# msyriac/orphics

Hardware: AMD Instinct MI355X
Metric: QE kappa reconstructions/sec on 8192^2 maps (higher is better)
Workload: dtype f64

## Files before the change

orphics_amd/csrc/common.hpp:

```cpp
#pragma once
#include <hip/hip_runtime.h>
#include <cstdio>
#include <cstring>
#include <string>
#include "../../include/orphics_amd.h"
#include "cx.hpp"

namespace oa {

std::string& last_error_ref();

inline int fail(const std::string& msg) {
    last_error_ref() = msg;
    return 1;
}

#define OA_HIP(expr)                                                                              \
    do {                                                                                          \
        hipError_t _e = (expr);                                                                   \
        if (_e != hipSuccess)                                                                     \
            return ::oa::fail(std::string(#expr) + ": " + hipGetErrorString(_e) + " (" + __FILE__ + \
                              ":" + std::to_string(__LINE__) + ")");                              \
    } while (0)

#define OA_REQUIRE(cond, msg)                         \
    do {                                              \
        if (!(cond)) return ::oa::fail(std::string(msg)); \
    } while (0)

#define OA_LAUNCH_CHECK() OA_HIP(hipGetLastError())

template <typename T, int N>
struct alignas(sizeof(T) * N > 16 ? 16 : sizeof(T) * N) Arr {
    T v[N];
};

struct DivBinFuse {
    const int32_t* ids; long ipitch;
    const int32_t* ids_t;
    const void* fn_t;
    int tab_logc, tab_rows;
    const unsigned long long* run_ent; const int32_t* run_off;
    int run_w, run_rb, run_cap;
    double pnorm; int nids, nxh;
    double* part;
    long part_cap;
    double* sums;
    unsigned* ticket;
    const int64_t* mcounts; int64_t* n; double* S; double* C;
    int store;
    int gx;
    bool done;
};

inline int flat_grid(long units, int block = 256, int cap = 8192) {
    long g = (units + block - 1) / block;
    if (g < 1) g = 1;
    if (g > cap) g = cap;
    return (int)g;
}

}

struct oa_plan {
    int ny, nx, logNy, logNx, dtype, device;
    long kp;
    void* tw_x;
    void* tw_y;
    void* scratch;
    size_t scratch_bytes;
    void* ly;
    void* lx;
    void* lyd;
    void* lxd;
    double* ly64;
    double* lx64;
    bool have_laxes;
    bool pow2;
    oa_plan* inner;
    int My, Mx;
    void* chirp_y; void* chirp_x;
    void* cz_bhat; void* cz_a; void* cz_f;
    void* cz_full;
    bool mixed;
    void* mr_twx; void* mr_twxh; void* mr_twy;
    void* pipe;
    void* rq8c[5];
    void* tw_y_small[16];
    void* tw_y_m3[16];
};

namespace oa {
int plan_ensure_scratch(oa_plan* p, size_t bytes);
int czt_setup(oa_plan* p);
void czt_release(oa_plan* p);
int czt_c2c(oa_plan* p, const void* in, void* out, int inverse, double scale, hipStream_t st);
int czt_r2c(oa_plan* p, const void* real_in, void* hc_out, double scale, hipStream_t st);
int czt_c2r(oa_plan* p, const void* hc_in, void* real_out, double scale, hipStream_t st);
bool mixed_sides_ok(int ny, int nx);
int mixed_setup(oa_plan* p);
void mixed_release(oa_plan* p);
int mixed_c2c(oa_plan* p, const void* in, void* out, int inverse, double scale, hipStream_t st);
int mixed_r2c(oa_plan* p, const void* real_in, void* hc_out, double scale, hipStream_t st);
int mixed_c2r(oa_plan* p, const void* hc_in, void* real_out, double scale, hipStream_t st);
int mixed_c2r_windowed(oa_plan* p, const void* hc_in, void* real_out, double scale, const void* window, hipStream_t st);
int mixed_cols_inverse(oa_plan* p, const void* hc_in, void* hc_out, hipStream_t st);
int mixed_lens_derivs(oa_plan* p, int nmaps, const void* real_in, long in_stride, void* k0, void* hc_pool, void* real_pool, int nd, hipStream_t st,
                      const void* hc_in, long hc_stride, double hc_scale);
void pipeline_release(oa_plan* p);
int n1_pool_reserve(oa_plan* p, size_t bytes, char** out);
long work_pitch(const oa_plan* p, int w);
int bin_power_moments(int dtype, const void* k, double norm, const int32_t* ids, long n, int nids, long hp, int nxh, double* sums,
                      int64_t* counts, void* scratch, int active_cols, int active_rows, unsigned* ticket,
                      const int64_t* mcounts, int64_t* mn, double* S, double* C, hipStream_t st, int nbatch = 1, long kstride = 0);
int stack_add_region(int dtype, const void* x, double* acc, int ny, long kp, int w, int rb, hipStream_t st, int nbatch = 1, long xstride = 0);
int band_rot2(int dtype, const void* c, const void* s, void* q, void* u, int ny, long kp, int w, int rb, hipStream_t st);
int stack_add_region_multi(int dtype, const void* k, long kstride, const void* wt, long wstride, int nest, double* const* acc, double* acc_mv,
                           int ny, long kp, int w, int rb, hipStream_t st);
int grf_mix_teb_to_tqu(oa_plan* p, uint64_t seed, uint64_t sid0, const void* const* cs, const void* rot_c, const void* rot_s, void* const* out,
                       hipStream_t st);
int band_stack_add_multi(int dtype, const void* k, long kstride, const void* wt, long wstride, int nest, double* const* acc, double* acc_mv,
                         int iny, long ipitch, int any, long apitch, int w, int r, hipStream_t st);
size_t rdn0_part_bytes(int ny, int rb, int nids, int B);
int rdn0_tail_check(const char* who, int nids, int B);
int rdn0_tail(int dtype, const void* k, long kstride, int B, int ny, long kp, int nxh, const int32_t* ids, int nids, double pnorm, int w, int rb,
              const int64_t* mcounts, double* part, int64_t* n, double* S, double* C, hipStream_t st);
size_t rdn0mv_scratch_bytes(int ny, int rb, int nspec, int nids);
int rdn0mv_tail_check(const char* who, int nest, bool have_w, int nspec, const int* host_a, const int* host_b, int nids);
int rdn0mv_tail(int dtype, const void* k, long kstride, const void* wt, long wstride, int nest, int nspec, const int* host_a, const int* host_b, int ny,
                long kp, int nxh, const int32_t* ids, int nids, double pnorm, int w, int rb, const int64_t* mcounts, void* scratch, int64_t* n, double* S,
                double* C, hipStream_t st);
// ... 78 lines not shown
```

orphics_amd/csrc/fft.hip:

```cpp
#include <algorithm>
#include <cmath>
#include <vector>
#include "fft_launch.hpp"
#include "fft_r2c_w64.hpp"
#include "fft_r2c_rs4096.hpp"
#include "fft_divbin.hpp"

namespace oa {

template <typename T, int MODE, class SEQ>
__global__ __launch_bounds__(row_maxnt<SEQ>(), waves_per_eu<T>()) void row_fft_kernel(RowArgs<T> a) {
    GpuCtx c{oa_dyn_smem};
    row_fft_body<T, MODE, SEQ>(c, a);
}

#ifndef OA_W64_OCC
#define OA_W64_OCC 1
#endif
__global__ __launch_bounds__(64, OA_W64_OCC) void row_r2c_w64_kernel(RowW64Args a) {
    GpuCtx c{oa_dyn_smem};
    row_r2c_w64_body(c, a);
}

template <typename T, class SEQ, int LR, bool PF>
// ... 387 lines not shown
        if (!ok && !rc) rc = fail("fft: unsupported row length");
    }
    template <typename T>
    void row_qe_pair8(int pairs, int M, const RowQeArgs<T>& a) {
        const bool ok = dispatch_rq8(M, a.win, a.lr, a.chain != nullptr, [&](auto ac, auto nzc, auto lay, auto ch) {
            constexpr int A = decltype(ac)::value;
            if (ch.value && !a.tab) { if (!rc) rc = fail("fft: estimator chains need a table"); return; }
            if (!a.rq8c) { if (!rc) rc = fail("fft: the 8-point row stage needs the constants of its grid"); return; }
            go(row_qe8_kernel<T, A, decltype(nzc)::value, decltype(lay)::value, decltype(ch)::value>, dim3(pairs), 64 * A, rq8_lds_bytes<T, A, decltype(ch)::value>(), a);
        });
        if (!ok && !rc) rc = fail("fft: unsupported row grid / layout for the 8-point row stage");
    }
    template <typename T>
    void row_qe_pair(int grid, int nt, size_t smem, const RowQeArgs<T>& a) {
        const bool ok = dispatch_seq(a.logL, [&](auto seq) {
            using S = decltype(seq);
            if constexpr (seq_logl<S>() >= 10 && seq_logl<S>() <= 13) {
                if (nt != pair_nt<S>()) { if (!rc) rc = fail("fft: pair row stage launched with the wrong workgroup size"); return; }
                dispatch_pair_nz<S>(pair_first_stage_nz(a.logL, S::rget(0), a.win), [&](auto nzc) {
                    if (a.chain) {
                        if constexpr (seq_logl<S>() <= 12) { if (a.lr == 0 && a.tab) go(row_qe_chain_kernel<T, S, decltype(nzc)::value>, dim3(grid), nt, smem, a); else if (!rc) rc = fail("fft: estimator chains need natural-order planes and a table"); }
                        else if (!rc) rc = fail("fft: estimator chains: unsupported row grid");
                    } else
                    if (a.lr == 2) go(row_qe_pair_kernel<T, S, decltype(nzc)::value, 2>, dim3(grid), nt, smem, a);
                    else if (a.lr == 3) {
                        if constexpr (seq_logl<S>() == 11 && sizeof(T) == 8) go(row_qe_pair_kernel<T, S, decltype(nzc)::value, 3>, dim3(grid), nt, smem, a);
                        else if (!rc) rc = fail("fft: the R = 8 layout of the pair row stage is built for float64 on 2048-point row grids");
                    } else if (a.lr == 0) go(row_qe_pair_kernel<T, S, decltype(nzc)::value, 0>, dim3(grid), nt, smem, a);
                    else if (!rc) rc = fail("fft: unsupported R-layout of the pair row stage");
                });
            } else if (!rc) rc = fail("fft: unsupported row grid for the pair row stage");
        });
        if (!ok && !rc) rc = fail("fft: unsupported row grid");
    }
    template <typename T>
    void col_legs(int gx, int gy, int nt, size_t smem, int logL, const ColLegsArgs<T>& a) {
        if (rc) return;
        rc = launch_col_legs<T>(st, gx, gy, nt, smem, logL, a);
    }
    template <typename T>
    void col_legs_sp(int gx, int nt, size_t smem, int logL, const ColLegsArgs<T>& a) {
        if (rc) return;
        rc = launch_col_legs_sp<T>(st, gx, nt, smem, logL, a);
    }
    template <typename T>
    void col_fwdlegs(int gx, int gy, int nt, size_t smem, int logL, const ColFwdLegsArgs<T>& a) {
        if (rc) return;
        rc = launch_col_fwdlegs<T>(st, gx, gy, nt, smem, logL, a);
    }
    template <typename T>
    void col_fwdlegs_cg(int gx, int gy, int nt, size_t smem, int logL, const ColFwdLegsCgArgs<T>& a, int gz = 1) {
        if (rc) return;
        rc = launch_col_fwdlegs_cg<T>(st, gx, gy, nt, smem, logL, a, gz);
    }
    template <typename T>
    void col_div(int gx, int gy, int nt, size_t smem, int logL, const ColDivArgs<T>& a, int gz = 1) {
        const bool ok = dispatch_seq(logL, [&](auto seq) {
            using S = decltype(seq);
            if constexpr (seq_logl<S>() <= 8) {
                if (nt > col_maxnt<S>()) { if (!rc) rc = fail("fft: column workgroup size exceeds its launch bound"); return; }
                go(col_div_kernel<T, S>, dim3(gx, gy, gz), nt, smem, a);
            } else if (!rc) rc = fail("fft: unsupported column sub-length");
        });
        if (!ok && !rc) rc = fail("fft: unsupported column length");
    }
    DivBinFuse* fuse = nullptr;
#define OA_GO_FUSED(K, ...) go_fused(K<__VA_ARGS__, false>, K<__VA_ARGS__, true>, gx, gz, nt, smem, a)
    template <class K, typename T>
    void go_fused(K kern_ids, K kern_runs, int gx, int gz, int nt, size_t smem, ColDivArgs<T> a) {
        const bool tabs = fuse->tab_logc == a.logC && fuse->tab_rows == a.ny;
        const bool runs = tabs && fuse->run_ent && fuse->run_w == a.width && fuse->run_rb == a.rband && fuse->run_cap <= 2 * nt;
        const K kern = runs ? kern_runs : kern_ids;
        if (runs) smem = std::max(smem, divrun_lds_bytes(a.ny, a.logC, nt, sizeof(T) == 8));
        {
            const hipError_t e = ensure_dyn_lds(reinterpret_cast<const void*>(kern), smem);
            if (e != hipSuccess) { rc = fail(std::string("hipFuncSetAttribute: ") + hipGetErrorString(e)); return; }
        }
        fuse->gx = gx;
        if (!fuse->store) a.out = nullptr;
        a.Fn_t = (tabs && a.fn_moff == 0) ? (const T*)fuse->fn_t : nullptr;
        if (!tabs) fuse->ids_t = nullptr;
        hipLaunchKernelGGL(kern, dim3(gx, 1, gz), dim3(nt), smem, st, a, *fuse);
        hipError_t e = hipGetLastError();
        if (e != hipSuccess) rc = fail(std::string("fft launch: ") + hipGetErrorString(e));
        fuse->done = true;
    }
    template <typename T>
    bool col_div_sp(int gx, size_t smem, int logL, const ColDivArgs<T>& a, int gz = 1) {
        if (rc) return true;
        const int lt = Fft2dPlan<T>::div_lt(), nt = (1 << lt) / EPT;
        const bool narrow = lt < (sizeof(T) == 4 ? 14 : 13);
        constexpr int lc11 = sizeof(T) == 4 ? 3 : 2, lc10 = lc11 + 1;
        if (fuse && !a.accumulate && (long)gx * gz * fuse->nids <= fuse->part_cap && (logL == 10 || logL == 11 || (logL == 12 && !narrow)) &&
            (size_t)(nt / 64) * fuse->nids * sizeof(double) <= ((size_t)1 << lt) * sizeof(cx<T>)) {
            if (logL == 12) OA_GO_FUSED(col_div_sp_bin_kernel, T, Seq<16, 16, 16>, lc11 - 1);
            else if (logL == 11 && !narrow) OA_GO_FUSED(col_div_sp_bin_kernel, T, Seq<16, 16, 8>, lc11);
            else if (logL == 10 && !narrow) OA_GO_FUSED(col_div_sp_bin_kernel, T, Seq<16, 16, 4>, lc10);
            else if (logL == 11) OA_GO_FUSED(col_div_sp_bin_kernel, T, Seq<16, 16, 8>, lc11 - 1);
            else OA_GO_FUSED(col_div_sp_bin_kernel, T, Seq<16, 16, 4>, lc10 - 1);
            return true;
        }
        if (logL == 12 && !narrow) { go(col_div_sp_kernel<T, Seq<16, 16, 16>, lc11 - 1>, dim3(gx, 1, gz), nt, smem, a); return true; }
        if (logL == 11 && !narrow) { go(col_div_sp_kernel<T, Seq<16, 16, 8>, lc11>, dim3(gx, 1, gz), nt, smem, a); return true; }
        if (logL == 10 && !narrow) { go(col_div_sp_kernel<T, Seq<16, 16, 4>, lc10>, dim3(gx, 1, gz), nt, smem, a); return true; }
        if (logL == 11) { go(col_div_sp_kernel<T, Seq<16, 16, 8>, lc11 - 1>, dim3(gx, 1, gz), nt, smem, a); return true; }
        if (logL == 10) { go(col_div_sp_kernel<T, Seq<16, 16, 4>, lc10 - 1>, dim3(gx, 1, gz), nt, smem, a); return true; }
        return false;
    }
    template <typename T>
    void col_div3(int gx, size_t smem, int rows, const ColDivArgs<T>& a, int gz = 1) {
        if (rc) return;
        constexpr int lc = sizeof(T) == 4 ? 3 : 2;
        if (rows != 1536 && rows != 768) { rc = fail("fft: unsupported 3 x 2^k divergence grid"); return; }
        const int nt = a.NT;
        if (fuse && !a.accumulate && (long)gx * gz * fuse->nids <= fuse->part_cap &&
            (size_t)(nt / 64) * fuse->nids * sizeof(double) <= ((size_t)rows << a.logC) * sizeof(cx<T>)) {
            if (rows == 1536) OA_GO_FUSED(col_div3_sp_bin_kernel, T, 8, lc);
            else OA_GO_FUSED(col_div3_sp_bin_kernel, T, 7, lc + 1);
            return;
        }
        if (rows == 1536) go(col_div3_sp_kernel<T, 8, lc>, dim3(gx, 1, gz), nt, smem, a);
        else go(col_div3_sp_kernel<T, 7, lc + 1>, dim3(gx, 1, gz), nt, smem, a);
    }
    template <typename T>
    void col_deriv(int gx, int gy, int nt, size_t smem, const ColDerivArgs<T>& a, int nz) {
        const bool ok = dispatch_seq(a.logL, [&](auto seq) {
            using S = decltype(seq);
            if constexpr (seq_logl<S>() <= 8) {
                if (nt > col_maxnt<S>()) { if (!rc) rc = fail("fft: column workgroup size exceeds its launch bound"); return; }
                go(col_deriv_kernel<T, S>, dim3(gx, gy, nz), nt, smem, a);
            } else if (!rc) rc = fail("fft: unsupported column sub-length");
        });
        if (!ok && !rc) rc = fail("fft: unsupported column length");
    }
    template <typename T>
    void col_grf(int gx, int gy, int nt, size_t smem, const GrfColArgs<T>& a, int nz) {
        const bool ok = dispatch_seq(a.logL, [&](auto seq) {
            using S = decltype(seq);
            if constexpr (seq_logl<S>() <= 8) {
                if (nt > col_maxnt<S>()) { if (!rc) rc = fail("fft: column workgroup size exceeds its launch bound"); return; }
                go(col_grf_kernel<T, S>, dim3(gx, gy, nz), nt, smem, a);
            } else if (!rc) rc = fail("fft: unsupported column sub-length");
        });
        if (!ok && !rc) rc = fail("fft: unsupported column length");
    }
    template <typename T>
    void col_mix(int gx, int gy, int nt, size_t smem, const MixColArgs<T>& a, int nz) {
        const bool ok = dispatch_seq(a.logL, [&](auto seq) {
            using S = decltype(seq);
            if constexpr (seq_logl<S>() <= 8 && !(sizeof(T) == 8 && seq_logl<S>() == 8)) {
                if (nt > col_maxnt<S>()) { if (!rc) rc = fail("fft: column workgroup size exceeds its launch bound"); return; }
                go(col_mix_kernel<T, S>, dim3(gx, gy, nz), nt, smem, a);
            } else if (!rc) rc = fail("fft: unsupported column sub-length");
        });
        if (!ok && !rc) rc = fail("fft: unsupported column length");
    }
    template <typename T>
    void col(int gx, int gy, int nt, size_t smem, const ColArgs<T>& a, int nz = 1) {
        const bool ok = dispatch_seq(a.logL, [&](auto seq) {
            using S = decltype(seq);
            if constexpr (seq_logl<S>() <= 8) {
                if (nt > col_maxnt<S>()) { if (!rc) rc = fail("fft: column workgroup size exceeds its launch bound"); return; }
                go(col_fft_kernel<T, S>, dim3(gx, gy, nz), nt, smem, a);
            } else {
                if (!rc) rc = fail("fft: unsupported column sub-length");
            }
// ... 689 lines not shown
```

orphics_amd/csrc/fft_divbin.hpp:

```cpp
#pragma once
#include "fft_launch.hpp"

namespace oa {

#if defined(__HIP_DEVICE_COMPILE__) && !(defined(__gfx942__) || defined(__gfx950__))
#error "DivBinTail: the ticket hand-over relies on gfx942 / gfx950 behaviour (agent-scope relaxed atomic stores are sc1 write-through, stores count in vmcnt)"
#endif

template <int CTRL>
__device__ __forceinline__ double dpp_f64(double v) {
    const unsigned long long u = __builtin_bit_cast(unsigned long long, v);
    const int lo = __builtin_amdgcn_update_dpp(0, (int)(unsigned)u, CTRL, 0xf, 0xf, false);
    const int hi = __builtin_amdgcn_update_dpp(0, (int)(unsigned)(u >> 32), CTRL, 0xf, 0xf, false);
    return __builtin_bit_cast(double, ((unsigned long long)(unsigned)hi << 32) | (unsigned long long)(unsigned)lo);
}
__device__ __forceinline__ double readlane_f64(double v, int lane) {
    const unsigned long long u = __builtin_bit_cast(unsigned long long, v);
    const unsigned lo = (unsigned)__builtin_amdgcn_readlane((int)(unsigned)u, lane);
    const unsigned hi = (unsigned)__builtin_amdgcn_readlane((int)(unsigned)(u >> 32), lane);
    return __builtin_bit_cast(double, ((unsigned long long)hi << 32) | (unsigned long long)lo);
}
__device__ __forceinline__ double wave_total_f64(double v) {
    v += dpp_f64<0xB1>(v);
    v += dpp_f64<0x4E>(v);
    v += dpp_f64<0x141>(v);
    v += dpp_f64<0x140>(v);
    return ((readlane_f64(v, 0) + readlane_f64(v, 16)) + readlane_f64(v, 32)) + readlane_f64(v, 48);
}

template <class Partial>
__device__ __forceinline__ void divbin_handover(const DivBinFuse& f, double* red, Partial partial) {
    __shared__ int s_last;
    const int t = threadIdx.x, nt = blockDim.x, nids = f.nids;
    const long wg = (long)blockIdx.z * gridDim.x + blockIdx.x;
    for (int i = t; i < nids; i += nt) {
        const double s = partial(i);
        __hip_atomic_store(f.part + wg * nids + i, s, __ATOMIC_RELAXED, __HIP_MEMORY_SCOPE_AGENT);
    }
    asm volatile("s_waitcnt vmcnt(0)" ::: "memory");
    __syncthreads();
    if (t == 0)
        s_last = (__hip_atomic_fetch_add(f.ticket, 1u, OA_TICKET_ORDER, __HIP_MEMORY_SCOPE_AGENT) == gridDim.x * gridDim.z - 1) ? 1 : 0;
    __syncthreads();
    if (!s_last) return;
    const int d = nids - 2;
    int NI = 1;
    while (NI < nids && NI < nt) NI <<= 1;
    const int G = nt / NI > 0 ? nt / NI : 1, gi = t / NI, ii = t - gi * NI;
    const int gx = (int)gridDim.x;
    for (int z = 0; z < (int)gridDim.z; ++z) {
        for (int i0 = 0; i0 < nids; i0 += NI) {
            const int i = i0 + ii;
            __syncthreads();
            if (gi < G) {
                double s = 0.0;
                if (i < nids) {
                    const double* pz = f.part + ((long)z * gx) * nids + i;
                    int b = gi;
                    for (; b + 3 * G < gx; b += 4 * G) {
                        const double p0 = __hip_atomic_load(pz + (long)b * nids, __ATOMIC_RELAXED, __HIP_MEMORY_SCOPE_AGENT);
                        const double p1 = __hip_atomic_load(pz + (long)(b + G) * nids, __ATOMIC_RELAXED, __HIP_MEMORY_SCOPE_AGENT);
                        const double p2 = __hip_atomic_load(pz + (long)(b + 2 * G) * nids, __ATOMIC_RELAXED, __HIP_MEMORY_SCOPE_AGENT);
                        const double p3 = __hip_atomic_load(pz + (long)(b + 3 * G) * nids, __ATOMIC_RELAXED, __HIP_MEMORY_SCOPE_AGENT);
                        s += (p0 + p1) + (p2 + p3);
                    }
                    for (; b < gx; b += G) s += __hip_atomic_load(pz + (long)b * nids, __ATOMIC_RELAXED, __HIP_MEMORY_SCOPE_AGENT);
                }
                red[gi * NI + ii] = s;
            }
            __syncthreads();
            double tot = 0.0;
            if (gi == 0 && i < nids) {
                for (int k = 0; k < G; ++k) tot += red[k * NI + ii];
                f.sums[(long)z * nids + i] = tot;
            }
            __syncthreads();
            if (gi == 0 && i >= 1 && i <= d) red[G * NI + i - 1] = tot / (double)f.mcounts[i];
        }
        __syncthreads();
        const double* bv = red + G * NI;
        if (f.S) {
            for (int a = t; a < d; a += nt) f.S[a] += bv[a];
            for (long e = t; e < (long)d * d; e += nt) {
                const int ra = (int)(e / d), cb = (int)(e - (long)ra * d);
                f.C[e] += bv[ra] * bv[cb];
            }
        }
    }
    if (t == 0) {
        if (f.n) f.n[0] += (int64_t)gridDim.z;
        __hip_atomic_store(f.ticket, 0u, __ATOMIC_RELAXED, __HIP_MEMORY_SCOPE_AGENT);
    }
}

template <typename T>
struct DivBinTail {
    static constexpr bool active = true, needs_ids = true;
    DivBinFuse f;
    double* rows = nullptr;

    __device__ __forceinline__ void begin(GpuCtx&, void* lds, int, int, int) {
        rows = reinterpret_cast<double*>(lds);
        const int nw = blockDim.x >> 6;
        for (int i = threadIdx.x; i < nw * f.nids; i += blockDim.x) rows[i] = 0.0;
    }
    __device__ __forceinline__ int id_at(unsigned yfull, int col) const { return f.ids[(long)yfull * f.ipitch + col]; }
    __device__ __forceinline__ bool packed_ids() const { return f.ids_t != nullptr; }
    __device__ __forceinline__ int id_at_t(long i) const { return f.ids_t[i]; }
    __device__ __forceinline__ void add(GpuCtx&, int id, T pw, int col, int) {
        const int m = (col == 0 || col == f.nxh) ? 1 : (col < f.nxh ? 2 : 0);
        const bool ok = id >= 0 && id < f.nids && m > 0;
        const double v = ok ? (double)(pw * (T)f.pnorm) * (double)m : 0.0;
        const int lane = threadIdx.x & 63;
        double* row = rows + (threadIdx.x >> 6) * f.nids;
        unsigned long long act = __ballot(ok);
        while (act) {
            const int leader = __ffsll((long long)act) - 1;
            const int lid = __shfl(id, leader, 64);
            const bool mine = ok && id == lid;
            const unsigned long long mm = __ballot(mine);
            const double sv = wave_total_f64(mine ? v : 0.0);
            if (lane == leader) row[lid] += sv;
            act &= ~mm;
        }
    }
    __device__ __forceinline__ void finish(GpuCtx&) {
        const int nw = blockDim.x >> 6, nids = f.nids;
        const double* r = rows;
        __syncthreads();
        divbin_handover(f, rows, [=](int i) {
            double s = 0.0;
            for (int k = 0; k < nw; ++k) s += r[k * nids + i];
            return s;
        });
    }
};

__host__ __device__ inline int divrun_col_stride(int rows, int logc) {
    const int want = (32 >> logc) > 0 ? (32 >> logc) : 1;
    const int s = rows + (rows >> 6) + 1;
    return s + (((want - s) % 32) + 32) % 32;
}
inline size_t divrun_lds_bytes(int rows, int logc, int nt, bool f64) {
    return ((size_t)divrun_col_stride(rows, logc) << logc) * sizeof(double) + (f64 ? (size_t)2 * nt * sizeof(double) : 0);
}
template <typename T>
struct DivRunTail {
    static constexpr bool active = true, needs_ids = false;
    static constexpr bool r_behind = sizeof(T) == 8;
    DivBinFuse f;
    double* P = nullptr;
    double* R = nullptr;
    const int32_t* offp = nullptr;
    int base = 0, cnt = 0, logc = 0, cs = 0, o0 = 0, o1 = 0;
    unsigned e0 = 0, e1 = 0;

    __device__ __forceinline__ void begin(GpuCtx&, void* lds, int tile, int logc_, int rows) {
        P = reinterpret_cast<double*>(lds);
        logc = logc_;
        cs = divrun_col_stride(rows, logc);
        R = r_behind ? P + ((long)cs << logc) : P;
        const int t = threadIdx.x, nt = blockDim.x;
        const int32_t* off = offp = f.run_off + (long)tile * (f.nids + 1);
        base = off[0];
        cnt = off[f.nids] - base;
        if (cnt > 2 * nt) cnt = 2 * nt;
        const unsigned* ew = reinterpret_cast<const unsigned*>(f.run_ent + base);
        e0 = t < cnt ? ew[2 * t] : 0u;
        e1 = t + nt < cnt ? ew[2 * (t + nt)] : 0u;
        if (t < f.nids) { o0 = off[t] - base; o1 = off[t + 1] - base; }
    }
    __device__ __forceinline__ int id_at(unsigned, int) const { return -1; }
    __device__ __forceinline__ bool packed_ids() const { return false; }
    __device__ __forceinline__ int id_at_t(long) const { return -1; }
    __device__ __forceinline__ void add(GpuCtx&, int, T pw, int col, int slot) {
        const int m = (col == 0 || col == f.nxh) ? 1 : (col < f.nxh ? 2 : 0);
        const int y = slot >> logc, c = slot & ((1 << logc) - 1);
        P[c * cs + y + (y >> 6)] = (double)(pw * (T)f.pnorm) * (double)m;
    }
    __device__ __forceinline__ double run_sum(unsigned w) const {
        const int first = (int)(w & 0xffffu), len = (int)((w >> 16) & 0xffu), col = (int)(w >> 24);
        const double* p = P + col * cs;
        double s = 0.0;
#pragma unroll 4
        for (int y = first; y < first + len; ++y) s += p[y + (y >> 6)];
        return s;
    }
    __device__ __forceinline__ void finish(GpuCtx&) {
        const int t = threadIdx.x, nt = blockDim.x;
        __syncthreads();
        const double s0 = run_sum(e0), s1 = run_sum(e1);
        if (!r_behind) __syncthreads();
        if (t < cnt) R[t] = s0;
        if (t + nt < cnt) R[t + nt] = s1;
        __syncthreads();
        const double* r = R;
        const int32_t* off = offp;
        const int a0 = o0, a1 = o1, b0 = base, n = cnt;
        divbin_handover(f, P, [=](int i) {
            int k = a0, k1 = a1;
            if (i != t) { k = off[i] - b0; k1 = off[i + 1] - b0; }
            if (k1 > n) k1 = n;
            double s = 0.0;
            for (; k < k1; ++k) s += r[k];
            return s;
        });
    }
};

}
```

orphics_amd/csrc/pipeline.hip:

```cpp
#include <dlfcn.h>
#include <cstdlib>
#include <algorithm>
#include <functional>
#include <string>
#include <utility>
#include <vector>
#include "common.hpp"
#include "fft_plan.hpp"
#include "divbin_runs.hpp"

namespace oa {

constexpr int MC_BATCH_MAX = 6;

struct DevBuf {
    void* p = nullptr;
    size_t bytes = 0;
    int reserve(size_t need, bool zero = false) {
        if (bytes >= need) return 0;
        if (p) { OA_HIP(hipDeviceSynchronize()); release(); }
        OA_HIP(hipMalloc(&p, need));
        bytes = need;
        if (zero) OA_HIP(hipMemset(p, 0, need));
        return 0;
// ... 373 lines not shown
        hipError_t e = hipMalloc(&z4, (size_t)p->ny * kp4 * es);
        if (e == hipSuccess) e = hipMemsetAsync(ids4, 0xFF, (size_t)p->ny * kp4 * sizeof(int32_t), (hipStream_t)stream);
        if (e == hipSuccess) e = hipMemsetAsync(z4, 0, (size_t)p->ny * kp4 * es, (hipStream_t)stream);
        if (e == hipSuccess)
            e = hipMemcpy2DAsync(ids4, kp4 * sizeof(int32_t), ids_hc, p->kp * sizeof(int32_t), p->kp * sizeof(int32_t), p->ny, hipMemcpyDeviceToDevice,
                                 (hipStream_t)stream);
        int rc = e == hipSuccess ? oa_bin_power(p->dtype, z4, z4, norm, ids4, nullptr, (long)p->ny * kp4, nids, kp4, p->nx / 2, q->sums, q->counts_full,
                                                nullptr, q->bin_scratch, 0, 0, stream)
                                 : fail(std::string("oa_plan_set_bins: padded bin ids: ") + hipGetErrorString(e));
        (void)hipStreamSynchronize((hipStream_t)stream);
        (void)hipFree(ids4);
        if (z4) (void)hipFree(z4);
        if (rc) return rc;
    }
    if (p->mixed) return (q->FG && q->band) ? mixed_bins(p, q, (hipStream_t)stream) : 0;
    return ensure_div_tables(p, q, (hipStream_t)stream);
}

void* oa_plan_kappa(oa_plan* p) { return (p && p->pipe) ? ((Pipeline*)p->pipe)->kk : nullptr; }
const int64_t* oa_plan_bin_counts(oa_plan* p) { return (p && p->pipe) ? ((Pipeline*)p->pipe)->counts_full : nullptr; }

static bool divbin_enabled(const Pipeline* q) { return q->opt_divbin; }
static int build_run_table(const oa_plan* p, Pipeline* q, Pipeline::DivTabs* t, int rows, int logc, long tiles, hipStream_t st) {
    t->has_runs = false;
    const int nxh = p->nx / 2;
    const int w = q->wk > nxh + 1 ? nxh + 1 : q->wk;
    const int rb = (q->rk <= 0 || 2L * q->rk - 1 >= rows) ? 0 : q->rk;
    const int cap = 2 * ((rows << logc) / 16);
    std::vector<int32_t> host((size_t)(tiles * rows) << logc);
    OA_HIP(hipMemcpyAsync(host.data(), t->ids_t.p, host.size() * 4, hipMemcpyDeviceToHost, st));
    OA_HIP(hipStreamSynchronize(st));
    DivRunTable tab;
    if (!divbin_build_runs(host.data(), (int)tiles, rows, logc, w, rb, q->nids, nxh, cap, &tab)) return 0;
    if (int rc = t->run_ent.reserve((tab.ent.size() + 1) * 8)) return rc;
    if (int rc = t->run_off.reserve(tab.off.size() * 4)) return rc;
    OA_HIP(hipMemcpyAsync(t->run_ent.p, tab.ent.data(), tab.ent.size() * 8, hipMemcpyHostToDevice, st));
    OA_HIP(hipMemcpyAsync(t->run_off.p, tab.off.data(), tab.off.size() * 4, hipMemcpyHostToDevice, st));
    OA_HIP(hipStreamSynchronize(st));
    t->has_runs = true; t->run_w = w; t->run_rb = rb; t->run_cap = cap;
    return 0;
}
static int ensure_div_tables(oa_plan* p, Pipeline* q, hipStream_t st, int rows) {
    Pipeline::DivTabs* const t = &q->tabs_of(rows);
    if (!(q->Fn && q->ids && (rows == 1024 || rows == 2048 || rows == 4096 || (q->my3 && rows == q->my3)) && q->wk > 0)) { t->tab_rows = 0; return 0; }
    const int logc = div_tile_logc(p, rows);
    if (t->tab_gen == q->bind_gen && t->tab_rows == rows && t->tab_logc == logc && t->tab_wk == q->wk) return 0;
    const size_t rs = p->dtype == OA_F32 ? 4 : 8;
    const long tiles = ((long)q->wk + (1 << logc) - 1) >> logc, total = (tiles * rows) << logc;
    if (int rc = t->fn_t.reserve((size_t)total * rs)) return rc;
    if (int rc = t->ids_t.reserve((size_t)total * 4)) return rc;
    if (int rc = pack_tiles(p, q->Fn, t->fn_t.p, rows, logc, q->wk, (int)rs, st)) return rc;
    if (int rc = pack_tiles(p, q->ids, t->ids_t.p, rows, logc, q->wk, 4, st)) return rc;
    if (int rc = build_run_table(p, q, t, rows, logc, tiles, st)) return rc;
    t->tab_gen = q->bind_gen; t->tab_rows = rows; t->tab_logc = logc; t->tab_wk = q->wk;
    return 0;
}
static int ensure_div_tables(oa_plan* p, Pipeline* q, hipStream_t st) {
    if (int rc = ensure_div_tables(p, q, st, q->my)) return rc;
    return q->my3 ? ensure_div_tables(p, q, st, q->my3) : 0;
}
static const void* fband_table(oa_plan* p, Pipeline* q, hipStream_t st) {
    static const bool off = exp_env("OA_NO_FBAND_TABLE") != nullptr;
    const int my = q->map_grid();
    if (off || !q->FG || my <= 0 || !qe_rsplit_lr(p, my, q->wl, q->wk, q->mrow)) return nullptr;
    if (q->fb_t.p && q->fb_gen == q->bind_gen && q->fb_my == my && q->fb_wl == q->wl && q->fb_rl == q->rl) return q->fb_t.p;
    if (q->fb_t.reserve((size_t)qe_fband_table_entries(p, q->wl, my) * elem_bytes(p))) { (void)hipGetLastError(); return nullptr; }
    if (qe_fband_pack_w(p, q->FG, q->FH, q->fb_t.p, q->wl, q->rl, my, st)) return nullptr;
    q->fb_gen = q->bind_gen; q->fb_my = my; q->fb_wl = q->wl; q->fb_rl = q->rl;
    return q->fb_t.p;
}
static DivBinFuse make_fuse(const oa_plan* p, const Pipeline* q, int64_t* n, double* S, double* C, int store, int rows = -1) {
    DivBinFuse f{};
    if (rows < 0) rows = q->my;
    const Pipeline::DivTabs& t = q->tabs_of(rows);
    if (t.tab_rows && t.tab_gen == q->bind_gen && t.tab_rows == rows && t.tab_wk == q->wk) {
        f.ids_t = (const int32_t*)t.ids_t.p; f.fn_t = t.fn_t.p; f.tab_logc = t.tab_logc; f.tab_rows = t.tab_rows;
        if (t.has_runs) {
            f.run_ent = (const unsigned long long*)t.run_ent.p; f.run_off = (const int32_t*)t.run_off.p;
            f.run_w = t.run_w; f.run_rb = t.run_rb; f.run_cap = t.run_cap;
        }
    }
    f.ids = q->ids; f.ipitch = p->kp; f.pnorm = q->norm; f.nids = q->nids; f.nxh = p->nx / 2;
    f.part = (double*)q->bin_scratch; f.part_cap = (long)(oa_bin_scratch_bytes(q->nids) / (long)sizeof(double)) * MC_BATCH_MAX;
    f.sums = q->sums; f.ticket = q->ticket; f.mcounts = q->counts_full; f.n = n; f.S = S; f.C = C; f.store = store; f.done = false;
    return f;
}

static int qe_tt_impl(oa_plan* p, const void* real_map, const void* kX, const void* kY, void* out_kappa_hc, int zero_outside,
                      void* stream, DivBinFuse* fuse, int rows_done = 0);
static int qe_mv_pow2(oa_plan* p, Pipeline* q, const MvCall& c, void* out, int accumulate, int leg_cols, int kappa_cols, int leg_rows,
                      int kappa_rows, int mrow, int zero_outside, hipStream_t st, bool keep_planes);
int oa_qe_tt(oa_plan* p, const void* real_map, const void* kX, const void* kY, void* out_kappa_hc, int zero_outside,
             void* stream) {
    if (p && p->mixed) {
        OA_REQUIRE(p->pipe && ((Pipeline*)p->pipe)->FG, "oa_qe_tt: call oa_plan_set_filters first");
        OA_REQUIRE((real_map != nullptr) != (kX != nullptr), "oa_qe_tt: pass either a real map or the Fourier-space leg(s)");
        return mixed_qe_tt(p, (Pipeline*)p->pipe, real_map, kX, kY, out_kappa_hc, zero_outside, (hipStream_t)stream);
    }
    return qe_tt_impl(p, real_map, kX, kY, out_kappa_hc, zero_outside, stream, nullptr);
}
static int qe_tt_impl(oa_plan* p, const void* real_map, const void* kX, const void* kY, void* out_kappa_hc, int zero_outside,
                      void* stream, DivBinFuse* fuse, int rows_done) {
    OA_REQUIRE(p && p->pipe && ((Pipeline*)p->pipe)->FG, "oa_qe_tt: call oa_plan_set_filters first");
    OA_REQUIRE((real_map != nullptr) != (kX != nullptr), "oa_qe_tt: pass either a real map or the Fourier-space leg(s)");
    Pipeline* q = (Pipeline*)p->pipe;
    void* out = out_kappa_hc ? out_kappa_hc : q->kk;
    if (out_kappa_hc && zero_outside)
        if (int rc = zero_complement(p, out, q->wk, q->rk, (hipStream_t)stream)) return rc;
    const long pl = work_pitch(p, q->wl), pk = work_pitch(p, q->wk);
    hipStream_t st = (hipStream_t)stream;
    int rc;
    const int my = (real_map && !rows_done) ? q->map_grid() : q->my;
    const int lr = (real_map && !rows_done) ? qe_rsplit_lr(p, my, q->wl, q->wk, q->mrow) : 0;
    if (real_map) rc = qe_map_legs_cols_w(p, real_map, q->FG, q->FH, q->c[0], q->c[1], q->c[2], q->wl, q->rl, pl, st, rows_done ? 6 : 7, my, lr,
                                          lr ? fband_table(p, q, st) : nullptr);
    else rc = qe_legs_cols_w(p, kX, kY ? kY : kX, q->FG, q->FH, q->c[0], q->c[1], q->c[2], q->wl, q->rl, pl, st, my);
    if (rc) return rc;
    const double s = 1.0 / ((double)p->ny * p->nx), sy = my ? (double)p->ny / my : 1.0;
    if ((rc = qe_rows_w(p, q->c[0], q->c[1], q->c[2], q->g[0], q->g[1], s * s * sy, 0, q->wl, q->wk, q->mrow, pl, pk, st, my, lr))) return rc;
    return qe_cols_div_w(p, q->g[0], q->g[1], q->Fn, out, 0, q->wk, q->rk, pk, st, my, fuse);
}

int oa_qe_pol(oa_plan* p, int npieces, const double* host_signs, const void* const* host_FG, const void* const* host_FH,
              const int* host_swap, const void* kX, const void* kY, const void* Fnorm, void* out, int accumulate,
              int leg_cols, int kappa_cols, int leg_rows, int kappa_rows, int mrow, int zero_outside, void* stream) {
    OA_REQUIRE(p && npieces >= 1 && host_signs && host_FG && host_FH && kX && kY && Fnorm && out, "oa_qe_pol: bad argument");
    OA_REQUIRE(p->pow2 || p->mixed, "oa_qe_pol: map sides with a prime factor other than 2, 3 and 5 (chirp-z transforms) have no one-call path "
               "(use the modular oa_qe_legs / oa_mul_real / oa_qe_div calls)");
    Pipeline* q = pipe_of(p);
    if (p->mixed) {
        const MvCall c{1, &npieces, host_signs, host_FG, host_FH, host_swap, &kX, &kY, &Fnorm, true};
        return mixed_qe_mv(p, q, c, out, accumulate, leg_cols, kappa_cols, leg_rows, kappa_rows, mrow, zero_outside, (hipStream_t)stream);
    }
    if (int rc = ensure_work(p, q)) return rc;
    if (!accumulate && zero_outside && out != q->kk)
        if (int rc = zero_complement(p, out, kappa_cols, kappa_rows, (hipStream_t)stream)) return rc;
    const long pl = work_pitch(p, leg_cols), pk = work_pitch(p, kappa_cols);
    hipStream_t st = (hipStream_t)stream;
    int my = 0;
    if (int rc = resolve_my(p, mrow == 0 ? 0 : q->mcol, leg_rows, kappa_rows, &my)) return rc;
    const double s = 1.0 / ((double)p->ny * p->nx), sy = my ? (double)p->ny / my : 1.0;
    for (int i = 0; i < npieces; ++i) {
        const bool sw = host_swap && host_swap[i];
        int rc = qe_legs_cols_w(p, sw ? kY : kX, sw ? kX : kY, host_FG[i], host_FH[i], q->c[0], q->c[1], q->c[2], leg_cols, leg_rows, pl, st, my);
        if (rc) return rc;
        if ((rc = qe_rows_w(p, q->c[0], q->c[1], q->c[2], q->g[0], q->g[1], host_signs[i] * s * s * sy, i > 0, leg_cols, kappa_cols, mrow, pl, pk, st, my))) return rc;
    }
    return qe_cols_div_w(p, q->g[0], q->g[1], Fnorm, out, accumulate, kappa_cols, kappa_rows, pk, st, my);
}

static int lens_maps_impl(oa_plan* p, int nmaps, const void* real_in, long in_stride, const void* hc_in, long hc_stride, double hc_scale, int order,
                          const int32_t* shift_x, const int32_t* shift_y, const void* dx, const void* dy, void* real_out, long out_stride, void* stream) {
    const long rplane = (long)p->ny * p->nx;
    Pipeline* q = pipe_of(p);
    const size_t rs = p->dtype == OA_F32 ? 4 : 8;
    const int nd = order * (order + 1) / 2 - 1;
    const int d00 = hc_in ? 1 : 0;
    hipStream_t st = (hipStream_t)stream;
    char* realp = nullptr;
    if (nd + d00 > 0) {
        const size_t hcb = plane_bytes(p), rb = (size_t)rplane * rs;
        const int chunk = 1;
        const size_t nk0 = hc_in ? 0 : (size_t)nmaps;
        if (int rc = q->lens_pool.reserve(nk0 * hcb + (size_t)chunk * hcb + (size_t)nmaps * (nd + d00) * rb)) return rc;
        char* k0 = q->lens_pool.at();
        char* hcp = k0 + nk0 * hcb;
        realp = hcp + (size_t)chunk * hcb;
// ... 1942 lines not shown
```

Before: 5930.

## Replace last-block ticket reduction with separate single-block fold kernel

Drops the atomic-ticket handover, in which the last finishing workgroup of the fused column-divide/bin kernel reduced every partial. Each workgroup now writes plain partial sums, and a separate one-block fold kernel sums them across workgroups and z-slices and updates S, C and n. The fold loop also loads 16 partials per iteration for more memory-level parallelism, and S/C/n are written once after all z-slices instead of once per slice. This removes agent-scope atomics, the vmcnt wait and the tail serialization in the main kernel, at the cost of an extra kernel launch and an LDS attribute call on every launch.

```diff
diff --git a/orphics_amd/csrc/common.hpp b/orphics_amd/csrc/common.hpp
--- a/orphics_amd/csrc/common.hpp
+++ b/orphics_amd/csrc/common.hpp
@@ -46,7 +46,6 @@
     double* part;
     long part_cap;
     double* sums;
-    unsigned* ticket;
     const int64_t* mcounts; int64_t* n; double* S; double* C;
     int store;
     int gx;
diff --git a/orphics_amd/csrc/fft.hip b/orphics_amd/csrc/fft.hip
--- a/orphics_amd/csrc/fft.hip
+++ b/orphics_amd/csrc/fft.hip
@@ -493,6 +493,14 @@
         if (!tabs) fuse->ids_t = nullptr;
         hipLaunchKernelGGL(kern, dim3(gx, 1, gz), dim3(nt), smem, st, a, *fuse);
         hipError_t e = hipGetLastError();
+        if (e == hipSuccess) {
+            const size_t fl = divbin_fold_lds_bytes(fuse->nids, nt, gz);
+            e = ensure_dyn_lds(reinterpret_cast<const void*>(divbin_fold_kernel), fl);
+            if (e == hipSuccess) {
+                hipLaunchKernelGGL(divbin_fold_kernel, dim3(1), dim3(nt), fl, st, *fuse, gz);
+                e = hipGetLastError();
+            }
+        }
         if (e != hipSuccess) rc = fail(std::string("fft launch: ") + hipGetErrorString(e));
         fuse->done = true;
     }
diff --git a/orphics_amd/csrc/fft_divbin.hpp b/orphics_amd/csrc/fft_divbin.hpp
--- a/orphics_amd/csrc/fft_divbin.hpp
+++ b/orphics_amd/csrc/fft_divbin.hpp
@@ -2,10 +2,6 @@
 #include "fft_launch.hpp"
 
 namespace oa {
-
-#if defined(__HIP_DEVICE_COMPILE__) && !(defined(__gfx942__) || defined(__gfx950__))
-#error "DivBinTail: the ticket hand-over relies on gfx942 / gfx950 behaviour (agent-scope relaxed atomic stores are sc1 write-through, stores count in vmcnt)"
-#endif
 
 template <int CTRL>
 __device__ __forceinline__ double dpp_f64(double v) {
@@ -29,68 +25,80 @@
 }
 
 template <class Partial>
-__device__ __forceinline__ void divbin_handover(const DivBinFuse& f, double* red, Partial partial) {
-    __shared__ int s_last;
-    const int t = threadIdx.x, nt = blockDim.x, nids = f.nids;
-    const long wg = (long)blockIdx.z * gridDim.x + blockIdx.x;
-    for (int i = t; i < nids; i += nt) {
-        const double s = partial(i);
-        __hip_atomic_store(f.part + wg * nids + i, s, __ATOMIC_RELAXED, __HIP_MEMORY_SCOPE_AGENT);
-    }
-    asm volatile("s_waitcnt vmcnt(0)" ::: "memory");
-    __syncthreads();
-    if (t == 0)
-        s_last = (__hip_atomic_fetch_add(f.ticket, 1u, OA_TICKET_ORDER, __HIP_MEMORY_SCOPE_AGENT) == gridDim.x * gridDim.z - 1) ? 1 : 0;
-    __syncthreads();
-    if (!s_last) return;
-    const int d = nids - 2;
+__device__ __forceinline__ void divbin_handover(const DivBinFuse& f, Partial partial) {
+    const int nids = f.nids;
+    double* mine = f.part + ((long)blockIdx.z * gridDim.x + blockIdx.x) * nids;
+    for (int i = threadIdx.x; i < nids; i += blockDim.x) mine[i] = partial(i);
+}
+
+__host__ __device__ inline int divbin_fold_ni(int nids, int nt) {
     int NI = 1;
-    while (NI < nids && NI < nt) NI <<= 1;
-    const int G = nt / NI > 0 ? nt / NI : 1, gi = t / NI, ii = t - gi * NI;
-    const int gx = (int)gridDim.x;
-    for (int z = 0; z < (int)gridDim.z; ++z) {
+    while (NI < nids && 2 * NI <= nt) NI <<= 1;
+    return NI;
+}
+inline size_t divbin_fold_lds_bytes(int nids, int nt, int gz) { return ((size_t)nt + (size_t)gz * nids) * sizeof(double); }
+
+__global__ __launch_bounds__(1024) void divbin_fold_kernel(DivBinFuse f, int gz) {
+    extern __shared__ double oa_fold_red[];
+    double* red = oa_fold_red;
+    const int t = threadIdx.x, nt = blockDim.x, nids = f.nids, d = nids - 2, gx = f.gx, dd = d * d;
+    const int NI = divbin_fold_ni(nids, nt);
+    const int G = nt / NI, gi = t / NI, ii = t - gi * NI;
+    double* bv = red + G * NI;
+    const bool mom = f.S != nullptr;
+    const double S0 = (mom && t < d) ? f.S[t] : 0.0, C0 = (mom && t < dd) ? f.C[t] : 0.0;
+    const int64_t n0 = (t == 0 && f.n) ? f.n[0] : 0;
+    for (int z = 0; z < gz; ++z) {
         for (int i0 = 0; i0 < nids; i0 += NI) {
             const int i = i0 + ii;
+            const bool isb = gi == 0 && i >= 1 && i <= d;
+            const int64_t mc = isb ? f.mcounts[i] : 1;
             __syncthreads();
             if (gi < G) {
                 double s = 0.0;
                 if (i < nids) {
                     const double* pz = f.part + ((long)z * gx) * nids + i;
-                    int b = gi;
-                    for (; b + 3 * G < gx; b += 4 * G) {
-                        const double p0 = __hip_atomic_load(pz + (long)b * nids, __ATOMIC_RELAXED, __HIP_MEMORY_SCOPE_AGENT);
-                        const double p1 = __hip_atomic_load(pz + (long)(b + G) * nids, __ATOMIC_RELAXED, __HIP_MEMORY_SCOPE_AGENT);
-                        const double p2 = __hip_atomic_load(pz + (long)(b + 2 * G) * nids, __ATOMIC_RELAXED, __HIP_MEMORY_SCOPE_AGENT);
-                        const double p3 = __hip_atomic_load(pz + (long)(b + 3 * G) * nids, __ATOMIC_RELAXED, __HIP_MEMORY_SCOPE_AGENT);
-                        s += (p0 + p1) + (p2 + p3);
+                    for (int b = gi; b < gx; b += 16 * G) {
+                        double p[16];
+#pragma unroll
+                        for (int k = 0; k < 16; ++k) p[k] = pz[(long)(b + k * G < gx ? b + k * G : gx - 1) * nids];
+#pragma unroll
+                        for (int j = 0; j < 16; j += 4) {
+                            if (b + (j + 3) * G < gx) s += (p[j] + p[j + 1]) + (p[j + 2] + p[j + 3]);
+                            else {
+#pragma unroll
+                                for (int k = j; k < j + 4; ++k)
+                                    if (b + k * G < gx) s += p[k];
+                            }
+                        }
                     }
-                    for (; b < gx; b += G) s += __hip_atomic_load(pz + (long)b * nids, __ATOMIC_RELAXED, __HIP_MEMORY_SCOPE_AGENT);
                 }
                 red[gi * NI + ii] = s;
             }
             __syncthreads();
-            double tot = 0.0;
             if (gi == 0 && i < nids) {
+                double tot = 0.0;
                 for (int k = 0; k < G; ++k) tot += red[k * NI + ii];
                 f.sums[(long)z * nids + i] = tot;
+                if (isb) bv[z * d + i - 1] = tot / (double)mc;
             }
-            __syncthreads();
-            if (gi == 0 && i >= 1 && i <= d) red[G * NI + i - 1] = tot / (double)f.mcounts[i];
-        }
-        __syncthreads();
-        const double* bv = red + G * NI;
-        if (f.S) {
-            for (int a = t; a < d; a += nt) f.S[a] += bv[a];
-            for (long e = t; e < (long)d * d; e += nt) {
-                const int ra = (int)(e / d), cb = (int)(e - (long)ra * d);
-                f.C[e] += bv[ra] * bv[cb];
-            }
-        }
-    }
-    if (t == 0) {
-        if (f.n) f.n[0] += (int64_t)gridDim.z;
-        __hip_atomic_store(f.ticket, 0u, __ATOMIC_RELAXED, __HIP_MEMORY_SCOPE_AGENT);
-    }
+        }
+    }
+    __syncthreads();
+    if (mom) {
+        for (int a = t; a < d; a += nt) {
+            double s = a == t ? S0 : f.S[a];
+            for (int z = 0; z < gz; ++z) s += bv[z * d + a];
+            f.S[a] = s;
+        }
+        for (int e = t; e < dd; e += nt) {
+            const int ra = e / d, cb = e - ra * d;
+            double c = e == t ? C0 : f.C[e];
+            for (int z = 0; z < gz; ++z) c += bv[z * d + ra] * bv[z * d + cb];
+            f.C[e] = c;
+        }
+    }
+    if (t == 0 && f.n) f.n[0] = n0 + (int64_t)gz;
 }
 
 template <typename T>
@@ -128,7 +136,7 @@
         const int nw = blockDim.x >> 6, nids = f.nids;
         const double* r = rows;
         __syncthreads();
-        divbin_handover(f, rows, [=](int i) {
+        divbin_handover(f, [=](int i) {
             double s = 0.0;
             for (int k = 0; k < nw; ++k) s += r[k * nids + i];
             return s;
@@ -197,7 +205,7 @@
         const double* r = R;
         const int32_t* off = offp;
         const int a0 = o0, a1 = o1, b0 = base, n = cnt;
-        divbin_handover(f, P, [=](int i) {
+        divbin_handover(f, [=](int i) {
             int k = a0, k1 = a1;
             if (i != t) { k = off[i] - b0; k1 = off[i + 1] - b0; }
             if (k1 > n) k1 = n;
diff --git a/orphics_amd/csrc/pipeline.hip b/orphics_amd/csrc/pipeline.hip
--- a/orphics_amd/csrc/pipeline.hip
+++ b/orphics_amd/csrc/pipeline.hip
@@ -479,7 +479,7 @@
     }
     f.ids = q->ids; f.ipitch = p->kp; f.pnorm = q->norm; f.nids = q->nids; f.nxh = p->nx / 2;
     f.part = (double*)q->bin_scratch; f.part_cap = (long)(oa_bin_scratch_bytes(q->nids) / (long)sizeof(double)) * MC_BATCH_MAX;
-    f.sums = q->sums; f.ticket = q->ticket; f.mcounts = q->counts_full; f.n = n; f.S = S; f.C = C; f.store = store; f.done = false;
+    f.sums = q->sums; f.mcounts = q->counts_full; f.n = n; f.S = S; f.C = C; f.store = store; f.done = false;
     return f;
 }
 
```

New measurement: 6061 (median of 6 runs). 1.02x the previous value.
